# dahiyaaneesh/peclr

Measured on AMD Instinct MI355X. Metric: images/sec (2-view) ResNet-50 bs128 @1/2/4/8 MI355X; NT-Xent loss Δ vs ref, higher is better.
Workload: dtype fp32; 1 GPU; ResNet-50 encoder, 2x128 synthetic 224x224 views per GPU, crop+rotate equivariance alignment, NT-Xent tau=0.5, LARS(Adam) step, fp32; global_batch=256, parallelism=dp1, accumulate_grad_batches=1, launch=one hipGraph replay per step (whole step captured), bn=per-rank batch statistics

## Files before the change

peclr_amd/csrc/stem.hip:

```cpp
#include <stdlib.h>

#include <type_traits>

#include "mfma.hpp"

namespace peclr {
namespace {

constexpr int SK = 14;
constexpr int TPX = 128;
constexpr int PWP = 2 * TPX + 6;
constexpr int PROW = PWP * 8;
constexpr int NROW = 9;
constexpr int XE = 68;

struct StemArgs {
    const float* x;
    const void* planes;
    void* y;
    int N, Hin, Win, Ho, Wo;
    int tiles_w;
    const float* stat_shift;
    float* stat_partial;
};

struct X6 {
    static constexpr int NP = 3;
    typedef float Out;
    static __device__ __forceinline__ f32x16 mma(const uint4& a, const uint4& b, f32x16 acc) { return mma_bf16(a, b, acc); }
};
struct HB : BF16 {
    static constexpr int NP = 1;
    typedef h16_t Out;
};
struct HF : F16 {
    static constexpr int NP = 1;
    typedef h16_t Out;
};

template <typename F>
__global__ __launch_bounds__(256, 2) void stem_fwd_kernel(StemArgs g) {
    constexpr int NP = F::NP;
    constexpr int PLANE = NROW * PROW;
    constexpr int CH = NP * 2 * 1024;
    constexpr int NB = 4;
    constexpr int B0 = 0, P0 = NB * CH;
    constexpr int EPI = 4 * 32 * XE * 4 + 4 * 2 * 64 * 4;
    constexpr int TOTAL = P0 + NP * PLANE > EPI ? P0 + NP * PLANE : EPI;
    __shared__ __attribute__((aligned(1024))) unsigned char lds[TOTAL];
    const int tid = threadIdx.x, lane = tid & 63, wave = tid >> 6;
    const int i = lane & 31, half = lane >> 5;
    typedef __attribute__((address_space(3))) unsigned char* lptr_t;
    const unsigned lds0 = __builtin_amdgcn_readfirstlane((unsigned)(__UINTPTR_TYPE__)(lptr_t)lds);
    const int wave_s = __builtin_amdgcn_readfirstlane(wave);

// ... 150 lines not shown
#pragma unroll
        for (int y = 0; y < 2; ++y)
#pragma unroll
            for (int r = 0; r < 16; ++r) wl[mfma32_row(r, half) * XE + y * 32 + i] = acc[a][y][r];
#pragma unroll
        for (int jj = 0; jj < 4; ++jj) {
            const int ow = wpx0 + er + 8 * jj;
            const float4 c0 = *reinterpret_cast<const float4*>(wl + (er + 8 * jj) * XE + ec);
            const float4 c1 = *reinterpret_cast<const float4*>(wl + (er + 8 * jj) * XE + ec + 4);
            if (oh < g.Ho && ow < g.Wo) {
                const size_t o = (((size_t)img * g.Ho + oh) * g.Wo + ow) * 64 + ec;
                if constexpr (NP == 3) {
                    float* out = static_cast<float*>(g.y) + o;
                    *reinterpret_cast<float4*>(out) = c0;
                    *reinterpret_cast<float4*>(out + 4) = c1;
                } else {
                    uint16_t* out = static_cast<uint16_t*>(g.y) + o;
                    *reinterpret_cast<uint4*>(out) = make_uint4(F::pack2(c0.x, c0.y), F::pack2(c0.z, c0.w), F::pack2(c1.x, c1.y), F::pack2(c1.z, c1.w));
                }
            }
        }
    }
}

__global__ __launch_bounds__(128) void stem_pack_kernel(const float* w, long sn, long sc, long sh, long sw, unsigned char* planes, int fmt) {
    const int t = blockIdx.x, y = threadIdx.x >> 6, l = threadIdx.x & 63;
    const int n = 32 * y + (l & 31), slice = 2 * t + (l >> 5), kh = slice >> 2, s = slice & 3;
    float v[8];
#pragma unroll
    for (int kk = 0; kk < 8; ++kk) {
        const int kw = 2 * s + (kk >> 2), c = kk & 3;
        v[kk] = (kw < 7 && c < 3) ? w[n * sn + c * sc + kh * sh + kw * sw] : 0.f;
    }
    if (fmt == 0) {
        unsigned h[4], m[4], lo[4];
#pragma unroll
        for (int q = 0; q < 4; ++q) split3_pk(v[2 * q], v[2 * q + 1], h[q], m[q], lo[q]);
        unsigned char* d = planes + (size_t)t * 6144 + (y * 3) * 1024 + l * 16;
        *reinterpret_cast<uint4*>(d) = make_uint4(h[0], h[1], h[2], h[3]);
        *reinterpret_cast<uint4*>(d + 1024) = make_uint4(m[0], m[1], m[2], m[3]);
        *reinterpret_cast<uint4*>(d + 2048) = make_uint4(lo[0], lo[1], lo[2], lo[3]);
    } else {
        unsigned q4[4];
#pragma unroll
        for (int q = 0; q < 4; ++q) q4[q] = fmt == 2 ? HF::pack2(v[2 * q], v[2 * q + 1]) : HB::pack2(v[2 * q], v[2 * q + 1]);
        *reinterpret_cast<uint4*>(planes + (size_t)t * 2048 + y * 1024 + l * 16) = make_uint4(q4[0], q4[1], q4[2], q4[3]);
    }
}


constexpr int WPX = 64;
constexpr int WPW = 2 * WPX + 6;
constexpr int WROW = WPW * 8;
constexpr int WAP = (WPX + 8) * 2;

struct StemWArgs {
    const float* x;
    const void* dy;
    float* slabs;
    int N, Hin, Win, Ho, Wo, tiles_w;
    long long tiles;
    int abl;
};

struct Gather {
    unsigned lo[4], hi[4];
};
template <int OFF>
__device__ __forceinline__ void gather8(unsigned addr, Gather& r) {
    asm volatile(
        "ds_read_u16 %0, %8 offset:%9\n\t"
        "ds_read_u16 %4, %8 offset:%10\n\t"
        "ds_read_u16 %1, %8 offset:%11\n\t"
        "ds_read_u16 %5, %8 offset:%12\n\t"
        "ds_read_u16 %2, %8 offset:%13\n\t"
        "ds_read_u16 %6, %8 offset:%14\n\t"
        "ds_read_u16 %3, %8 offset:%15\n\t"
        "ds_read_u16 %7, %8 offset:%16"
        : "=v"(r.lo[0]), "=v"(r.lo[1]), "=v"(r.lo[2]), "=v"(r.lo[3]), "=v"(r.hi[0]), "=v"(r.hi[1]), "=v"(r.hi[2]), "=v"(r.hi[3])
        : "v"(addr), "n"(OFF), "n"(OFF + 16), "n"(OFF + 32), "n"(OFF + 48), "n"(OFF + 64), "n"(OFF + 80), "n"(OFF + 96), "n"(OFF + 112)
        : "memory");
}
template <int NP>
__device__ __forceinline__ void gather_fence(Gather (&g)[NP]) {
    if constexpr (NP == 3) {
        asm volatile("s_waitcnt lgkmcnt(0)"
                     : "+v"(g[0].lo[0]), "+v"(g[0].lo[1]), "+v"(g[0].lo[2]), "+v"(g[0].lo[3]), "+v"(g[0].hi[0]), "+v"(g[0].hi[1]),
                       "+v"(g[0].hi[2]), "+v"(g[0].hi[3]), "+v"(g[1].lo[0]), "+v"(g[1].lo[1]), "+v"(g[1].lo[2]), "+v"(g[1].lo[3]),
                       "+v"(g[1].hi[0]), "+v"(g[1].hi[1]), "+v"(g[1].hi[2]), "+v"(g[1].hi[3]), "+v"(g[2].lo[0]), "+v"(g[2].lo[1]),
                       "+v"(g[2].lo[2]), "+v"(g[2].lo[3]), "+v"(g[2].hi[0]), "+v"(g[2].hi[1]), "+v"(g[2].hi[2]), "+v"(g[2].hi[3])
                     :: "memory");
    } else {
        asm volatile("s_waitcnt lgkmcnt(0)"
                     : "+v"(g[0].lo[0]), "+v"(g[0].lo[1]), "+v"(g[0].lo[2]), "+v"(g[0].lo[3]), "+v"(g[0].hi[0]), "+v"(g[0].hi[1]),
                       "+v"(g[0].hi[2]), "+v"(g[0].hi[3])
                     :: "memory");
    }
}
__device__ __forceinline__ uint4 merge(const Gather& g) {
    return make_uint4(g.lo[0] | (g.hi[0] << 16), g.lo[1] | (g.hi[1] << 16), g.lo[2] | (g.hi[2] << 16), g.lo[3] | (g.hi[3] << 16));
}

template <typename F>
__global__ __launch_bounds__(256, F::NP == 3 ? 2 : 3) void stem_wgrad_kernel(StemWArgs g) {
    constexpr int NP = F::NP;
    constexpr int PPL = 7 * WROW;
    constexpr int APL = 64 * WAP;
    constexpr int STAGE = NP * (PPL + APL);
    constexpr int NST = NP == 3 ? 1 : 2;
    __shared__ __attribute__((aligned(16))) unsigned char lds[NST * STAGE];
    const int tid = threadIdx.x, lane = tid & 63, wave = tid >> 6;
    const int i = lane & 31, half = lane >> 5;
    typedef __attribute__((address_space(3))) unsigned char* lptr_t;
    const unsigned lds0 = (unsigned)(__UINTPTR_TYPE__)(lptr_t)lds;
    const int nkh = wave == 3 ? 1 : 2;

    f32x16 acc[2][2];
#pragma unroll
    for (int a = 0; a < 2; ++a)
#pragma unroll
        for (int b = 0; b < 2; ++b)
#pragma unroll
            for (int r = 0; r < 16; ++r) acc[a][b][r] = 0.f;

    constexpr int NSLOT = 7 * WPW, NLD = (NSLOT + 255) / 256;
    struct __attribute__((packed, aligned(4))) Rgb { float r, g, b; };
    Rgb pxs[2][NLD];
    constexpr int NDY = NP == 3 ? 4 : 2;
    uint4 dyrs[2][NDY];
    auto tile_of = [&](long long t64, int& img, int& oh, int& ow0) {
        const int per_img = g.Ho * g.tiles_w, t = (int)t64;
        img = t / per_img;
        const int rem = t - img * per_img;
        oh = rem / g.tiles_w;
        ow0 = (rem - oh * g.tiles_w) * WPX;
    };
    auto gload = [&](long long t, Rgb (&px)[NLD], uint4 (&dyr)[NDY]) {
        int img, oh, ow0;
        tile_of(t, img, oh, ow0);
        const int ih0 = 2 * oh - 3, iw0 = 2 * ow0 - 3;
#pragma unroll
        for (int u = 0; u < NLD; ++u) {
            const int idx = tid + 256 * u;
            const int r = idx / WPW, p = idx - r * WPW;
            const int ih = ih0 + r, iw = iw0 + p;
            const bool in = idx < NSLOT && (unsigned)ih < (unsigned)g.Hin && (unsigned)iw < (unsigned)g.Win;
            const Rgb* src = reinterpret_cast<const Rgb*>(g.x + (((size_t)img * g.Hin + (in ? ih : 0)) * g.Win + (in ? iw : 0)) * 3);
            px[u] = (in && !(g.abl & 16)) ? *src : Rgb{0.f, 0.f, 0.f};
        }
        const size_t row0 = ((size_t)img * g.Ho + oh) * g.Wo;
#pragma unroll
        for (int u = 0; u < NDY; ++u) {
            const int p = NP == 3 ? 16 * u + (lane & 15) : 32 * u + (lane & 31);
            const int grp = NP == 3 ? 4 * wave + (lane >> 4) : 2 * wave + (lane >> 5);
            const bool live = ow0 + p < g.Wo;
            const size_t row = row0 + (live ? ow0 + p : 0);
            const uint4* src = NP == 3 ? reinterpret_cast<const uint4*>(static_cast<const float*>(g.dy) + row * 64 + 4 * grp)
                                       : reinterpret_cast<const uint4*>(static_cast<const uint16_t*>(g.dy) + row * 64 + 8 * grp);
            if (live && !(g.abl & 1)) {
                if (g.abl & 32) {
                    const u32x4 t = __builtin_nontemporal_load(reinterpret_cast<const u32x4*>(src));
                    dyr[u] = make_uint4(t[0], t[1], t[2], t[3]);
                } else dyr[u] = *src;
            } else dyr[u] = make_uint4(0u, 0u, 0u, 0u);
        }
    };
    auto stage_store = [&](int st, const Rgb (&px)[NLD], const uint4 (&dyr)[NDY]) {
        unsigned char* base = lds + st * STAGE;
#pragma unroll
        for (int u = 0; u < NLD; ++u) {
            const int idx = tid + 256 * u;
            if (idx < NSLOT) {
                unsigned char* d = base + idx * 8;
                if constexpr (NP == 3) {
                    unsigned h[2], m[2], l[2];
                    split3_pk(px[u].r, px[u].g, h[0], m[0], l[0]);
                    split3_pk(px[u].b, 0.f, h[1], m[1], l[1]);
                    *reinterpret_cast<uint2*>(d) = make_uint2(h[0], h[1]);
                    *reinterpret_cast<uint2*>(d + PPL) = make_uint2(m[0], m[1]);
                    *reinterpret_cast<uint2*>(d + 2 * PPL) = make_uint2(l[0], l[1]);
                } else {
                    *reinterpret_cast<uint2*>(d) = make_uint2(F::pack2(px[u].r, px[u].g), F::pack2(px[u].b, 0.f));
                }
            }
        }
        unsigned char* ab = base + NP * PPL;
        if (g.abl & 2) return;
#pragma unroll
        for (int u = 0; u < NDY; ++u) {
            const int p = NP == 3 ? 16 * u + (lane & 15) : 32 * u + (lane & 31);
            const int grp = NP == 3 ? 4 * wave + (lane >> 4) : 2 * wave + (lane >> 5);
            if constexpr (NP == 3) {
                const unsigned w[4] = {dyr[u].x, dyr[u].y, dyr[u].z, dyr[u].w};
                unsigned h[2], m[2], l[2];
                split3_pk(__uint_as_float(w[0]), __uint_as_float(w[1]), h[0], m[0], l[0]);
                split3_pk(__uint_as_float(w[2]), __uint_as_float(w[3]), h[1], m[1], l[1]);
#pragma unroll
                for (int q = 0; q < 4; ++q) {
                    unsigned short* d = reinterpret_cast<unsigned short*>(ab + (4 * grp + q) * WAP + p * 2);
                    const int sh = (q & 1) * 16;
                    d[0] = (unsigned short)(h[q >> 1] >> sh);
                    d[APL / 2] = (unsigned short)(m[q >> 1] >> sh);
                    d[APL] = (unsigned short)(l[q >> 1] >> sh);
                }
            } else {
                const unsigned w[4] = {dyr[u].x, dyr[u].y, dyr[u].z, dyr[u].w};
#pragma unroll
                for (int q = 0; q < 8; ++q)
                    *reinterpret_cast<unsigned short*>(ab + (8 * grp + q) * WAP + p * 2) = (unsigned short)(w[q >> 1] >> ((q & 1) * 16));
            }
        }
    };

    const unsigned bbase = 2 * i + 128 * half + (2 * wave) * WROW;
    const unsigned abase = NP * PPL + i * WAP + 16 * half;

    auto products = [&](int st) {
        const unsigned sb = lds0 + st * STAGE;
        const unsigned char* sa = lds + st * STAGE + abase;
#pragma unroll
        for (int ks = 0; ks < WPX / 16; ++ks) {
            uint4 af[2][NP], bf[2][NP];
            Gather gb[2][NP];
#pragma unroll
            for (int p = 0; p < NP; ++p)
#pragma unroll
                for (int q = 0; q < 4; ++q) gb[1][p].lo[q] = gb[1][p].hi[q] = 0u;
#pragma unroll
            for (int mt = 0; mt < 2; ++mt)
#pragma unroll
                for (int p = 0; p < NP; ++p) af[mt][p] = *reinterpret_cast<const uint4*>(sa + p * APL + mt * 32 * WAP + ks * 32);
            auto row = [&](auto kc, int b) {
                constexpr int KO = decltype(kc)::value * 256;
                const unsigned addr = sb + bbase + b * WROW;
                gather8<KO>(addr, gb[b][0]);
                if constexpr (NP == 3) {
                    gather8<PPL + KO>(addr, gb[b][1]);
                    gather8<2 * PPL + KO>(addr, gb[b][2]);
                }
            };
            auto both = [&](auto kc) { row(kc, 0); if (nkh == 2) row(kc, 1); };
            if (g.abl & 4) { }
            else if (ks == 0) both(std::integral_constant<int, 0>{});
            else if (ks == 1) both(std::integral_constant<int, 1>{});
            else if (ks == 2) both(std::integral_constant<int, 2>{});
            else both(std::integral_constant<int, 3>{});
            gather_fence<NP>(gb[0]);
            gather_fence<NP>(gb[1]);
#pragma unroll
            for (int b = 0; b < 2; ++b)
#pragma unroll
                for (int p = 0; p < NP; ++p) bf[b][p] = merge(gb[b][p]);
#pragma unroll
            for (int b = 0; b < 2; ++b) {
                if (b < nkh && !(g.abl & 8)) {
#pragma unroll
                    for (int mt = 0; mt < 2; ++mt) {
                        if constexpr (NP == 3) {
                            acc[mt][b] = F::mma(af[mt][2], bf[b][0], acc[mt][b]);
                            acc[mt][b] = F::mma(af[mt][0], bf[b][2], acc[mt][b]);
                            acc[mt][b] = F::mma(af[mt][1], bf[b][1], acc[mt][b]);
                            acc[mt][b] = F::mma(af[mt][1], bf[b][0], acc[mt][b]);
                            acc[mt][b] = F::mma(af[mt][0], bf[b][1], acc[mt][b]);
                            acc[mt][b] = F::mma(af[mt][0], bf[b][0], acc[mt][b]);
                        } else {
                            acc[mt][b] = F::mma(af[mt][0], bf[b][0], acc[mt][b]);
                        }
                    }
                }
            }
        }
    };
    const long long step = gridDim.x;
    long long t = blockIdx.x;
    if (t < g.tiles) {
        gload(t, pxs[0], dyrs[0]);
        if (t + step < g.tiles) gload(t + step, pxs[1], dyrs[1]);
        stage_store(0, pxs[0], dyrs[0]);
    }
    __syncthreads();
    int st = 0;
    while (t < g.tiles) {
#pragma unroll
        for (int cur = 1; cur >= 0; --cur) {
            if (t < g.tiles) {
                if (t + 2 * step < g.tiles) gload(t + 2 * step, pxs[cur ^ 1], dyrs[cur ^ 1]);
                products(st);
                if constexpr (NST == 1) __syncthreads();
                if (t + step < g.tiles) stage_store(st ^ (NST - 1), pxs[cur], dyrs[cur]);
                __syncthreads();
                t += step;
                st ^= (NST - 1);
            }
        }
    }
    float* slab = g.slabs + (size_t)blockIdx.x * 64 * 224;
#pragma unroll
    for (int b = 0; b < 2; ++b) {
        if (b < nkh) {
            const int kh = 2 * wave + b;
#pragma unroll
            for (int mt = 0; mt < 2; ++mt)
#pragma unroll
                for (int r = 0; r < 16; ++r) slab[(size_t)(32 * mt + mfma32_row(r, half)) * 224 + 32 * kh + i] = acc[mt][b][r];
        }
// ... 81 lines not shown
```

peclr_amd/csrc/gemm_x6t.hip:

```cpp
#include "mfma.hpp"

#include <type_traits>

namespace peclr {
namespace {

constexpr int TK = 16;

struct X6TArgs {
    const float* A;
    const float* B;
    float* slabs;
    int M, N, K, lda, ldb, ldc;
    int kchunk;
    int taps, H, W;
    int stride;
    const float* zeros;
};

__device__ __forceinline__ int slot_of(int i) { return (i & 3) * 8 + ((i >> 2) ^ (((i >> 1) & 1) << 2)); }

template <int MT, int NT, int WGM, bool GEO, int PF>
__global__ __launch_bounds__(512, 2) void gemm_x6t_kernel(X6TArgs g) {
    constexpr int WGN = 8 / WGM;
// ... 245 lines not shown
        split_store(0);
        if (nk > 1) gload(1);
    }
    __syncthreads();
    for (int t = 0; t < nk; ++t) {
        const unsigned char* bufp = lds + (t & 1) * BUF;
        uint4 af[3];
#pragma unroll
        for (int p = 0; p < 3; ++p) af[p] = *reinterpret_cast<const uint4*>(bufp + fa + p * 2048);
#pragma unroll
        for (int tp = 0; tp < NACC; ++tp) {
            if (WGM == 4 || tp < ntap) {
                uint4 bf[3];
#pragma unroll
                for (int p = 0; p < 3; ++p) bf[p] = *reinterpret_cast<const uint4*>(bufp + fb + tp * GRP + p * 2048);
                acc[tp] = mma_bf16(af[2], bf[0], acc[tp]);
                acc[tp] = mma_bf16(af[0], bf[2], acc[tp]);
                acc[tp] = mma_bf16(af[1], bf[1], acc[tp]);
                acc[tp] = mma_bf16(af[1], bf[0], acc[tp]);
                acc[tp] = mma_bf16(af[0], bf[1], acc[tp]);
                acc[tp] = mma_bf16(af[0], bf[0], acc[tp]);
            }
            if (tp == (WGM == 4 ? 2 : 1) && t + 1 < nk) {
                if constexpr (!(ABL & 4)) split_store((t + 1) & 1);
                if constexpr (!(ABL & 8)) if (t + 2 < nk) gload(t + 2);
            }
        }
        __syncthreads();
    }

    float* out = g.slabs + (size_t)blockIdx.y * g.M * g.ldc;
    float* wlds = reinterpret_cast<float*>(lds) + wave * (32 * XEPL);
    const int er = lane >> 3, ec = (lane & 7) * 4;
    const int mt = m0 + wm * 32, nt = n0 + wn * 32;
#pragma unroll
    for (int tp = 0; tp < NACC; ++tp) {
        if (WGM != 4 && tp >= ntap) break;
#pragma unroll
        for (int r = 0; r < 16; ++r) wlds[mfma32_row(r, kh) * XEPL + i] = acc[tp][r];
#pragma unroll
        for (int jj = 0; jj < 4; ++jj) {
            const int m = mt + er + 8 * jj, n = nt + ec;
            const float4 c = *reinterpret_cast<const float4*>(wlds + (er + 8 * jj) * XEPL + ec);
            if (m < g.M && n < g.N) *reinterpret_cast<float4*>(out + (size_t)m * g.ldc + (tap0 + tp) * g.N + n) = c;
        }
    }
}

constexpr int X6W2_MAX_HW = 3136;
constexpr int X6W2_TAB = 9 * X6W2_MAX_HW + 192;
constexpr int X6W2_S2_MAX_HW = X6W2_TAB / 36 - 3;


template <int WGM, bool S2 = false>
__global__ __launch_bounds__(512, 2) void gemm_x6w2_kernel(X6TArgs g) {
    constexpr int GRP = 3 * 2 * 64 * 16;
    constexpr int NGA = WGM / 2, NG = NGA + 9, BUF = NG * GRP;
    constexpr int NACC = WGM == 4 ? 9 : 5;
    constexpr int XEPL = 36;
    __shared__ __attribute__((aligned(1024))) unsigned char lds[2 * BUF + X6W2_TAB];
    unsigned char* const tab = lds + 2 * BUF;
    const int tid = threadIdx.x, lane = tid & 63;
    const int wave = __builtin_amdgcn_readfirstlane(tid >> 6);
    const int wm = WGM == 4 ? wave >> 1 : (wave >> 1) & 1, wn = wave & 1;
    const int tap0 = WGM == 4 ? 0 : (wave >> 2) * 5;
    const int ntap = WGM == 4 ? 9 : (wave >> 2 ? 4 : 5);
    const int i = lane & 31, kh = lane >> 5;
    const int nct = (g.N + 63) / 64;
    const int m0 = (int)(blockIdx.x / nct) * (32 * WGM), n0 = (int)(blockIdx.x % nct) * 64;
    const int kbeg = blockIdx.y * g.kchunk, kend = min(g.K, kbeg + g.kchunk);
    const int nk = (kend - kbeg + TK - 1) / TK;
    const int HW = g.H * g.W;

    const unsigned s2_ld4 = (unsigned)g.ldb * 4u, s2_img = 4u * HW * s2_ld4;
    const int s2_row = (HW + 3) * 4;
    if constexpr (S2) {
        unsigned* t32 = reinterpret_cast<unsigned*>(tab);
        for (int p = tid; p < HW; p += 512) {
            const int oh = p / g.W, ow = p - oh * g.W;
#pragma unroll
            for (int tap = 0; tap < 9; ++tap) {
                const int ih = 2 * oh + tap / 3 - 1, iw = 2 * ow + tap % 3 - 1;
                const bool in = ih >= 0 && iw >= 0;
                const unsigned e = in ? (unsigned)(ih * 2 * g.W + iw) * s2_ld4 : 0x40000000u;
                t32[tap * (HW + 3) + p] = e;
                if (p < 3) t32[tap * (HW + 3) + HW + p] = in ? e + s2_img : 0x40000000u;
            }
        }
        __syncthreads();
    } else {

        unsigned short* pm = reinterpret_cast<unsigned short*>(lds);
        for (int p = tid; p < HW; p += 512) {
            const int oh = p / g.W, ow = p - oh * g.W;
            const unsigned rv = (oh > 0 ? 1u : 0u) | 2u | (oh + 1 < g.H ? 4u : 0u), cv = (ow > 0 ? 1u : 0u) | 2u | (ow + 1 < g.W ? 4u : 0u);
            unsigned bits = 0;
#pragma unroll
            for (int tap = 0; tap < 9; ++tap) bits |= ((rv >> (tap / 3)) & (cv >> (tap % 3)) & 1u) << tap;
            pm[p] = (unsigned short)bits;
        }
        __syncthreads();
        for (int p = tid; p < HW; p += 512) {
            unsigned v[4];
#pragma unroll
            for (int q = 0; q < 4; ++q) v[q] = pm[p + q < HW ? p + q : p + q - HW];
#pragma unroll
            for (int tap = 0; tap < 9; ++tap)
                tab[tap * X6W2_MAX_HW + p] = (unsigned char)(((v[0] >> tap) & 1u) | ((v[1] >> tap) & 1u) << 1 | ((v[2] >> tap) & 1u) << 2 | ((v[3] >> tap) & 1u) << 3);
        }
        __syncthreads();
    }

    const int chunk = (lane & 7) + 8 * (lane >> 5), kq = (lane >> 3) & 3;
    const int cin = 4 * (chunk & 7), tile = chunk >> 3;
    const int st_off = (kq >> 1) * 1024 + tile * 512 + (kq & 1) * 8;
    struct Grp {
        __amdgpu_buffer_rsrc_t rs;
        unsigned off;
        unsigned step, ld4;
        int tb;
        int st;
        bool isx;
    };
    auto grp_of = [&](int gi) {
        Grp s;
        const bool is_a = gi < NGA;
        const int tap = is_a ? 4 : gi - NGA;
        const int shift = (tap / 3 - 1) * g.W + (tap % 3 - 1);
        const int ld = is_a ? g.lda : g.ldb;
        const int c = 4 * chunk + (is_a ? 64 * gi : 0);
        const bool ok = is_a ? m0 + c < g.M : n0 + c < g.N;
        const long rows = S2 ? (is_a ? (long)g.K : 4L * g.K) : (long)g.K + (shift < 0 ? shift : 0);
        const unsigned long long bp = reinterpret_cast<unsigned long long>(is_a ? g.A : g.B);
        const unsigned blo = __builtin_amdgcn_readfirstlane((unsigned)bp), bhi = __builtin_amdgcn_readfirstlane((unsigned)(bp >> 32));
        s.rs = __builtin_amdgcn_make_buffer_rsrc(reinterpret_cast<void*>((unsigned long long)bhi << 32 | blo), (short)0,
                                                 __builtin_amdgcn_readfirstlane((int)(rows * ld * 4)), 0x00020000);
        s.ld4 = __builtin_amdgcn_readfirstlane((unsigned)ld * 4u);
        s.step = TK * s.ld4;
        s.off = ok ? (unsigned)(((kbeg + 4 * kq + shift) * ld + (is_a ? m0 : n0) + c) * 4) : 0x80000000u;
        s.tb = __builtin_amdgcn_readfirstlane(2 * BUF + tap * X6W2_MAX_HW);
        s.isx = !is_a;
        if constexpr (S2) {
            if (!is_a) s.off = ok ? (unsigned)((kbeg + 4 * kq) / HW) * s2_img + (unsigned)(n0 + c) * 4u : 0x80000000u;
            s.tb = __builtin_amdgcn_readfirstlane(2 * BUF + tap * s2_row);
        }
        s.st = gi * GRP + st_off;
        return s;
    };
    Grp G1 = grp_of(wave), G2 = grp_of(wave + 8 < NG ? wave + 8 : wave);
    const bool two = wave + 8 < NG;
    int pk = (kbeg + 4 * kq) % HW;

    f32x4 la[4], lb[4];
    unsigned m1 = 0, m2 = 0;
    auto issue_row = [&](const Grp& G, unsigned msk, int q, f32x4 (&r)[4]) {
        unsigned o;
        if constexpr (S2) o = G.off + (G.isx ? msk : q * G.ld4);
        else o = (msk >> q) & 1u ? G.off + q * G.ld4 : 0x80000000u;
        r[q] = __builtin_bit_cast(f32x4, __builtin_amdgcn_raw_buffer_load_b128(G.rs, (int)o, 0, 0));
    };
    auto entry = [&](const Grp& G, int q) { return *reinterpret_cast<const unsigned*>(lds + G.tb + 4 * (pk + q)); };
    auto issue = [&](const Grp& G, unsigned msk, int qp, f32x4 (&r)[4]) {
        if constexpr (S2) {
            issue_row(G, entry(G, 2 * qp), 2 * qp, r);
            issue_row(G, entry(G, 2 * qp + 1), 2 * qp + 1, r);
        } else {
            issue_row(G, msk, 2 * qp, r);
            issue_row(G, msk, 2 * qp + 1, r);
        }
    };
    unsigned winc = 0;
    auto next_pixel = [&]() {
        pk += TK;
        if constexpr (S2) winc = pk >= HW ? s2_img : 0u;
        pk = pk >= HW ? pk - HW : pk;
    };
    auto advance = [&](Grp& G) {
        if constexpr (S2) G.off += G.isx ? winc : G.step;
        else G.off += G.step;
    };
    struct Quarter { unsigned h, m; float r0, r1; };
    auto q_first = [&](Quarter& s, int qp, int j, const f32x4 (&r)[4]) {
        const float x0 = r[2 * qp][j], x1 = r[2 * qp + 1][j];
        s.h = pk_bf16(x0, x1);
        s.r0 = sub_f32(x0, __uint_as_float(s.h << 16));
        s.r1 = sub_f32(x1, __uint_as_float(s.h & 0xFFFF0000u));
    };
    auto q_second = [&](Quarter& s) {
        s.m = pk_bf16(s.r0, s.r1);
        s.r0 = sub_f32(s.r0, __uint_as_float(s.m << 16));
        s.r1 = sub_f32(s.r1, __uint_as_float(s.m & 0xFFFF0000u));
    };
    auto q_third = [&](const Quarter& s, const Grp& G, int buf, int qp, int j) {
        unsigned char* d = lds + G.st + buf * BUF + 4 * qp + slot_of(cin + j) * 16;
        *reinterpret_cast<unsigned*>(d) = s.h;
        *reinterpret_cast<unsigned*>(d + 2048) = s.m;
        *reinterpret_cast<unsigned*>(d + 4096) = pk_bf16(s.r0, s.r1);
    };
    auto quarter = [&](const Grp& G, int buf, int qp, int j, const f32x4 (&r)[4]) {
        Quarter s;
        q_first(s, qp, j, r);
        q_second(s);
        q_third(s, G, buf, qp, j);
    };

    f32x16 acc[NACC];
#pragma unroll
    for (int tp = 0; tp < NACC; ++tp)
#pragma unroll
        for (int r = 0; r < 16; ++r) acc[tp][r] = 0.f;
    const int fa = (wm >> 1) * GRP + kh * 1024 + (wm & 1) * 512 + slot_of(i) * 16;
    const int fb = (NGA + tap0) * GRP + kh * 1024 + wn * 512 + slot_of(i) * 16;

    __syncthreads();
    if constexpr (!S2) { m1 = lds[G1.tb + pk]; m2 = lds[G2.tb + pk]; }
    issue(G1, m1, 0, la); issue(G1, m1, 1, la);
    if (two) { issue(G2, m2, 0, lb); issue(G2, m2, 1, lb); }
    next_pixel(); advance(G1); advance(G2);
#pragma unroll
    for (int qp = 0; qp < 2; ++qp)
#pragma unroll
        for (int j = 0; j < 4; ++j) {
            quarter(G1, 0, qp, j, la);
            if (two) quarter(G2, 0, qp, j, lb);
        }
    if constexpr (!S2) { m1 = lds[G1.tb + pk]; m2 = lds[G2.tb + pk]; }
    issue(G1, m1, 0, la); issue(G1, m1, 1, la);
    if (two) { issue(G2, m2, 0, lb); issue(G2, m2, 1, lb); }
    next_pixel(); advance(G1); advance(G2);
    __syncthreads();

    auto run = [&](auto two_c) {
        constexpr bool TWO = decltype(two_c)::value;
        for (int t = 0; t < nk; ++t) {
            const unsigned char* bufp = lds + (t & 1) * BUF;
            const int nb = (t + 1) & 1;
            uint4 af[3], b0[2], b1, b2;
#pragma unroll
            for (int p = 0; p < 3; ++p) af[p] = *reinterpret_cast<const uint4*>(bufp + fa + p * 2048);
            b0[0] = *reinterpret_cast<const uint4*>(bufp + fb);
            b1 = *reinterpret_cast<const uint4*>(bufp + fb + 2048);
            b2 = *reinterpret_cast<const uint4*>(bufp + fb + 4096);
            const unsigned n1 = S2 ? 0u : lds[G1.tb + pk], n2 = (!S2 && TWO) ? lds[G2.tb + pk] : 0u;
            unsigned tq[2] = {0u, 0u};
#pragma unroll
            for (int tp = 0; tp < NACC; ++tp) {
                if (WGM != 4 && tp >= ntap) break;
                const int cb = tp & 1;
                const bool more = tp + 1 < NACC;
                const unsigned char* nx = bufp + fb + (tp + 1) * GRP;
                constexpr int PER = WGM == 4 ? 2 : 4;
                Quarter qs[PER];
                auto piece = [&](int e) {
                    const int u = PER * tp + e / 3, k = e % 3;
                    if (u >= (TWO ? 16 : 8)) return;
                    const int qp = (u >> 2) & 1, j = u & 3;
                    Quarter& s = qs[e / 3];
                    if (u < 8) {
                        if (k == 0) { q_first(s, qp, j, la); if (S2 && j == 2) { tq[0] = entry(G1, 2 * qp); tq[1] = entry(G1, 2 * qp + 1); } }
                        else if (k == 1) { q_second(s); if (j == 3) issue_row(G1, S2 ? tq[0] : n1, 2 * qp, la); }
                        else { q_third(s, G1, nb, qp, j); if (j == 3) issue_row(G1, S2 ? tq[1] : n1, 2 * qp + 1, la); }
                    } else {
                        if (k == 0) { q_first(s, qp, j, lb); if (S2 && j == 2) { tq[0] = entry(G2, 2 * qp); tq[1] = entry(G2, 2 * qp + 1); } }
                        else if (k == 1) { q_second(s); if (j == 3) issue_row(G2, S2 ? tq[0] : n2, 2 * qp, lb); }
                        else { q_third(s, G2, nb, qp, j); if (j == 3) issue_row(G2, S2 ? tq[1] : n2, 2 * qp + 1, lb); }
                    }
                };
                auto slot = [&](int si) {
                    if (WGM == 4) piece(si);
                    else { piece(2 * si); piece(2 * si + 1); }
                };
#define PECLR_FENCE __builtin_amdgcn_sched_barrier(0)
                acc[tp] = mma_bf16(af[2], b0[cb], acc[tp]);       PECLR_FENCE;
                if (more) b0[cb ^ 1] = *reinterpret_cast<const uint4*>(nx);
                slot(0);                                      PECLR_FENCE;
                acc[tp] = mma_bf16(af[0], b2, acc[tp]);           PECLR_FENCE;
                if (more) b2 = *reinterpret_cast<const uint4*>(nx + 4096);
                slot(1);                                      PECLR_FENCE;
                acc[tp] = mma_bf16(af[1], b1, acc[tp]);           PECLR_FENCE;
                slot(2);                                      PECLR_FENCE;
                acc[tp] = mma_bf16(af[1], b0[cb], acc[tp]);       PECLR_FENCE;
                slot(3);                                      PECLR_FENCE;
                acc[tp] = mma_bf16(af[0], b1, acc[tp]);           PECLR_FENCE;
                if (more) b1 = *reinterpret_cast<const uint4*>(nx + 2048);
                slot(4);                                      PECLR_FENCE;
                acc[tp] = mma_bf16(af[0], b0[cb], acc[tp]);       PECLR_FENCE;
                slot(5);                                      PECLR_FENCE;
#undef PECLR_FENCE
            }
            next_pixel();
            advance(G1);
            if (TWO) advance(G2);
            __syncthreads();
        }
    };
    if (two) run(std::true_type{});
    else run(std::false_type{});

    float* out = g.slabs + (size_t)blockIdx.y * g.M * g.ldc;
    float* wlds = reinterpret_cast<float*>(lds) + wave * (32 * XEPL);
    const int er = lane >> 3, ec = (lane & 7) * 4;
    const int mt = m0 + wm * 32, nt = n0 + wn * 32;
#pragma unroll
    for (int tp = 0; tp < NACC; ++tp) {
        if (WGM != 4 && tp >= ntap) break;
#pragma unroll
        for (int r = 0; r < 16; ++r) wlds[mfma32_row(r, kh) * XEPL + i] = acc[tp][r];
#pragma unroll
        for (int jj = 0; jj < 4; ++jj) {
            const int m = mt + er + 8 * jj, n = nt + ec;
            const float4 c = *reinterpret_cast<const float4*>(wlds + (er + 8 * jj) * XEPL + ec);
            if (m < g.M && n < g.N) *reinterpret_cast<float4*>(out + (size_t)m * g.ldc + (tap0 + tp) * g.N + n) = c;
        }
    }
}

template <int MT, int NT, int WGM, bool PF2 = false>
__global__ __launch_bounds__(512, 2) void gemm_x6t2_kernel(X6TArgs g) {
    constexpr int WGN = 8 / WGM;
    constexpr int TM = 32 * WGM * MT, TN = 32 * WGN * NT;
    static_assert((TM + TN) / 64 <= 8 && TM % 64 == 0 && TN % 64 == 0, "one 64-column group of the split per wave");
    constexpr int HALF_A = TM * 16, HALF_B = TN * 16;
    constexpr int PL_A = 2 * HALF_A, PL_B = 2 * HALF_B;
    constexpr int BUF = 3 * (PL_A + PL_B);
    constexpr int XEPL = 36;
    static_assert(2 * BUF >= 8 * 32 * XEPL * 4, "epilogue transposes live in the plane buffers");
    __shared__ __attribute__((aligned(1024))) unsigned char lds[2 * BUF];
    const int tid = threadIdx.x, lane = tid & 63;
    const int wave = __builtin_amdgcn_readfirstlane(tid >> 6);
    const int wm = wave / WGN, wn = wave % WGN;
    const int i = lane & 31, kh = lane >> 5;
    const int nct = (g.N + TN - 1) / TN;
    const int m0 = (int)(blockIdx.x / nct) * TM, n0 = (int)(blockIdx.x % nct) * TN;
    const int kbeg = blockIdx.y * g.kchunk, kend = min(g.K, kbeg + g.kchunk);
    const int nk = (kend - kbeg + TK - 1) / TK;

    const bool is_a = wave < TM / 64;
    const bool active = wave < (TM + TN) / 64;
    const int cgrp = is_a ? wave : wave - TM / 64;
    const int chunk = (lane & 7) + 8 * (lane >> 5);
    const int kq = (lane >> 3) & 3;
    const int col = cgrp * 64 + 4 * chunk;
    const int ld = is_a ? g.lda : g.ldb;
    const bool col_ok = active && (is_a ? m0 + col < g.M : n0 + col < g.N);
    const int tile = col >> 5, cin = col & 31;
    const int st_base = (kq >> 1) * (is_a ? HALF_A : HALF_B) + tile * 512 + (kq & 1) * 8 + (is_a ? 0 : 3 * PL_A);
    const int st_plane = is_a ? PL_A : PL_B;
    const bool once = is_a ? nct == 1 : (int)gridDim.x == nct;

    const unsigned long long bp = reinterpret_cast<unsigned long long>(is_a ? g.A : g.B);
// ... 248 lines not shown
```

Baseline: 5697 images/sec.

## Use ds_read_tr16 transposed LDS reads for stem wgrad fragments

Replaces the per-element ds_read_u16 gathers and merge for the pixel (B) fragments with ds_read_b64_tr_b16 transposing loads. It also changes the dy staging layout to pixel-major rows, written with wide vector stores instead of scattered 16-bit stores, and re-pads the A pitch. The intent is to cut LDS instruction count and the cost of scattered stores in the stem weight-gradient kernel. It relies on the gfx950 transpose-read builtin and a new lane-to-fragment mapping that must match the MFMA operand layout exactly.

```diff
diff --git a/peclr_amd/csrc/stem.hip b/peclr_amd/csrc/stem.hip
--- a/peclr_amd/csrc/stem.hip
+++ b/peclr_amd/csrc/stem.hip
@@ -1,6 +1,4 @@
 #include <stdlib.h>
-
-#include <type_traits>
 
 #include "mfma.hpp"
 
@@ -257,7 +255,7 @@
 constexpr int WPX = 64;
 constexpr int WPW = 2 * WPX + 6;
 constexpr int WROW = WPW * 8;
-constexpr int WAP = (WPX + 8) * 2;
+constexpr int WAP = 64 * 2 + 64;
 
 struct StemWArgs {
     const float* x;
@@ -268,56 +266,25 @@
     int abl;
 };
 
-struct Gather {
-    unsigned lo[4], hi[4];
-};
-template <int OFF>
-__device__ __forceinline__ void gather8(unsigned addr, Gather& r) {
-    asm volatile(
-        "ds_read_u16 %0, %8 offset:%9\n\t"
-        "ds_read_u16 %4, %8 offset:%10\n\t"
-        "ds_read_u16 %1, %8 offset:%11\n\t"
-        "ds_read_u16 %5, %8 offset:%12\n\t"
-        "ds_read_u16 %2, %8 offset:%13\n\t"
-        "ds_read_u16 %6, %8 offset:%14\n\t"
-        "ds_read_u16 %3, %8 offset:%15\n\t"
-        "ds_read_u16 %7, %8 offset:%16"
-        : "=v"(r.lo[0]), "=v"(r.lo[1]), "=v"(r.lo[2]), "=v"(r.lo[3]), "=v"(r.hi[0]), "=v"(r.hi[1]), "=v"(r.hi[2]), "=v"(r.hi[3])
-        : "v"(addr), "n"(OFF), "n"(OFF + 16), "n"(OFF + 32), "n"(OFF + 48), "n"(OFF + 64), "n"(OFF + 80), "n"(OFF + 96), "n"(OFF + 112)
-        : "memory");
-}
-template <int NP>
-__device__ __forceinline__ void gather_fence(Gather (&g)[NP]) {
-    if constexpr (NP == 3) {
-        asm volatile("s_waitcnt lgkmcnt(0)"
-                     : "+v"(g[0].lo[0]), "+v"(g[0].lo[1]), "+v"(g[0].lo[2]), "+v"(g[0].lo[3]), "+v"(g[0].hi[0]), "+v"(g[0].hi[1]),
-                       "+v"(g[0].hi[2]), "+v"(g[0].hi[3]), "+v"(g[1].lo[0]), "+v"(g[1].lo[1]), "+v"(g[1].lo[2]), "+v"(g[1].lo[3]),
-                       "+v"(g[1].hi[0]), "+v"(g[1].hi[1]), "+v"(g[1].hi[2]), "+v"(g[1].hi[3]), "+v"(g[2].lo[0]), "+v"(g[2].lo[1]),
-                       "+v"(g[2].lo[2]), "+v"(g[2].lo[3]), "+v"(g[2].hi[0]), "+v"(g[2].hi[1]), "+v"(g[2].hi[2]), "+v"(g[2].hi[3])
-                     :: "memory");
-    } else {
-        asm volatile("s_waitcnt lgkmcnt(0)"
-                     : "+v"(g[0].lo[0]), "+v"(g[0].lo[1]), "+v"(g[0].lo[2]), "+v"(g[0].lo[3]), "+v"(g[0].hi[0]), "+v"(g[0].hi[1]),
-                       "+v"(g[0].hi[2]), "+v"(g[0].hi[3])
-                     :: "memory");
-    }
-}
-__device__ __forceinline__ uint4 merge(const Gather& g) {
-    return make_uint4(g.lo[0] | (g.hi[0] << 16), g.lo[1] | (g.hi[1] << 16), g.lo[2] | (g.hi[2] << 16), g.lo[3] | (g.hi[3] << 16));
+typedef short s16x4 __attribute__((ext_vector_type(4)));
+template <int PITCH>
+__device__ __forceinline__ uint4 tr_frag(const unsigned char* base) {
+    typedef __attribute__((address_space(3))) s16x4* lp;
+    const uint2 lo = __builtin_bit_cast(uint2, __builtin_amdgcn_ds_read_tr16_b64_v4i16((lp)(base)));
+    const uint2 hi = __builtin_bit_cast(uint2, __builtin_amdgcn_ds_read_tr16_b64_v4i16((lp)(base + 4 * PITCH)));
+    return make_uint4(lo.x, lo.y, hi.x, hi.y);
 }
 
 template <typename F>
 __global__ __launch_bounds__(256, F::NP == 3 ? 2 : 3) void stem_wgrad_kernel(StemWArgs g) {
     constexpr int NP = F::NP;
     constexpr int PPL = 7 * WROW;
-    constexpr int APL = 64 * WAP;
+    constexpr int APL = WPX * WAP;
     constexpr int STAGE = NP * (PPL + APL);
     constexpr int NST = NP == 3 ? 1 : 2;
     __shared__ __attribute__((aligned(16))) unsigned char lds[NST * STAGE];
     const int tid = threadIdx.x, lane = tid & 63, wave = tid >> 6;
     const int i = lane & 31, half = lane >> 5;
-    typedef __attribute__((address_space(3))) unsigned char* lptr_t;
-    const unsigned lds0 = (unsigned)(__UINTPTR_TYPE__)(lptr_t)lds;
     const int nkh = wave == 3 ? 1 : 2;
 
     f32x16 acc[2][2];
@@ -356,8 +323,8 @@
         const size_t row0 = ((size_t)img * g.Ho + oh) * g.Wo;
 #pragma unroll
         for (int u = 0; u < NDY; ++u) {
-            const int p = NP == 3 ? 16 * u + (lane & 15) : 32 * u + (lane & 31);
-            const int grp = NP == 3 ? 4 * wave + (lane >> 4) : 2 * wave + (lane >> 5);
+            const int p = NP == 3 ? 16 * u + 4 * wave + (lane >> 4) : 32 * u + 8 * wave + (lane >> 3);
+            const int grp = NP == 3 ? lane & 15 : lane & 7;
             const bool live = ow0 + p < g.Wo;
             const size_t row = row0 + (live ? ow0 + p : 0);
             const uint4* src = NP == 3 ? reinterpret_cast<const uint4*>(static_cast<const float*>(g.dy) + row * 64 + 4 * grp)
@@ -393,69 +360,44 @@
         if (g.abl & 2) return;
 #pragma unroll
         for (int u = 0; u < NDY; ++u) {
-            const int p = NP == 3 ? 16 * u + (lane & 15) : 32 * u + (lane & 31);
-            const int grp = NP == 3 ? 4 * wave + (lane >> 4) : 2 * wave + (lane >> 5);
+            const int p = NP == 3 ? 16 * u + 4 * wave + (lane >> 4) : 32 * u + 8 * wave + (lane >> 3);
+            const int grp = NP == 3 ? lane & 15 : lane & 7;
             if constexpr (NP == 3) {
                 const unsigned w[4] = {dyr[u].x, dyr[u].y, dyr[u].z, dyr[u].w};
                 unsigned h[2], m[2], l[2];
                 split3_pk(__uint_as_float(w[0]), __uint_as_float(w[1]), h[0], m[0], l[0]);
                 split3_pk(__uint_as_float(w[2]), __uint_as_float(w[3]), h[1], m[1], l[1]);
-#pragma unroll
-                for (int q = 0; q < 4; ++q) {
-                    unsigned short* d = reinterpret_cast<unsigned short*>(ab + (4 * grp + q) * WAP + p * 2);
-                    const int sh = (q & 1) * 16;
-                    d[0] = (unsigned short)(h[q >> 1] >> sh);
-                    d[APL / 2] = (unsigned short)(m[q >> 1] >> sh);
-                    d[APL] = (unsigned short)(l[q >> 1] >> sh);
-                }
+                unsigned char* d = ab + p * WAP + grp * 8;
+                *reinterpret_cast<uint2*>(d) = make_uint2(h[0], h[1]);
+                *reinterpret_cast<uint2*>(d + APL) = make_uint2(m[0], m[1]);
+                *reinterpret_cast<uint2*>(d + 2 * APL) = make_uint2(l[0], l[1]);
             } else {
-                const unsigned w[4] = {dyr[u].x, dyr[u].y, dyr[u].z, dyr[u].w};
-#pragma unroll
-                for (int q = 0; q < 8; ++q)
-                    *reinterpret_cast<unsigned short*>(ab + (8 * grp + q) * WAP + p * 2) = (unsigned short)(w[q >> 1] >> ((q & 1) * 16));
+                *reinterpret_cast<uint4*>(ab + p * WAP + grp * 16) = dyr[u];
             }
         }
     };
 
-    const unsigned bbase = 2 * i + 128 * half + (2 * wave) * WROW;
-    const unsigned abase = NP * PPL + i * WAP + 16 * half;
+    const int fpix = 8 * half + ((lane & 15) >> 2), fcol = 2 * (16 * ((lane >> 4) & 1) + 4 * (lane & 3));
+    const unsigned bbase = fpix * 16 + fcol + (2 * wave) * WROW;
+    const unsigned abase = NP * PPL + fpix * WAP + fcol;
 
     auto products = [&](int st) {
-        const unsigned sb = lds0 + st * STAGE;
+        const unsigned char* sb = lds + st * STAGE + bbase;
         const unsigned char* sa = lds + st * STAGE + abase;
 #pragma unroll
         for (int ks = 0; ks < WPX / 16; ++ks) {
             uint4 af[2][NP], bf[2][NP];
-            Gather gb[2][NP];
-#pragma unroll
-            for (int p = 0; p < NP; ++p)
-#pragma unroll
-                for (int q = 0; q < 4; ++q) gb[1][p].lo[q] = gb[1][p].hi[q] = 0u;
 #pragma unroll
             for (int mt = 0; mt < 2; ++mt)
 #pragma unroll
-                for (int p = 0; p < NP; ++p) af[mt][p] = *reinterpret_cast<const uint4*>(sa + p * APL + mt * 32 * WAP + ks * 32);
-            auto row = [&](auto kc, int b) {
-                constexpr int KO = decltype(kc)::value * 256;
-                const unsigned addr = sb + bbase + b * WROW;
-                gather8<KO>(addr, gb[b][0]);
-                if constexpr (NP == 3) {
-                    gather8<PPL + KO>(addr, gb[b][1]);
-                    gather8<2 * PPL + KO>(addr, gb[b][2]);
+                for (int p = 0; p < NP; ++p) af[mt][p] = tr_frag<WAP>(sa + p * APL + mt * 64 + ks * 16 * WAP);
+#pragma unroll
+            for (int b = 0; b < 2; ++b)
+#pragma unroll
+                for (int p = 0; p < NP; ++p) {
+                    bf[b][p] = make_uint4(0u, 0u, 0u, 0u);
+                    if (b < nkh && !(g.abl & 4)) bf[b][p] = tr_frag<16>(sb + p * PPL + b * WROW + ks * 256);
                 }
-            };
-            auto both = [&](auto kc) { row(kc, 0); if (nkh == 2) row(kc, 1); };
-            if (g.abl & 4) { }
-            else if (ks == 0) both(std::integral_constant<int, 0>{});
-            else if (ks == 1) both(std::integral_constant<int, 1>{});
-            else if (ks == 2) both(std::integral_constant<int, 2>{});
-            else both(std::integral_constant<int, 3>{});
-            gather_fence<NP>(gb[0]);
-            gather_fence<NP>(gb[1]);
-#pragma unroll
-            for (int b = 0; b < 2; ++b)
-#pragma unroll
-                for (int p = 0; p < NP; ++p) bf[b][p] = merge(gb[b][p]);
 #pragma unroll
             for (int b = 0; b < 2; ++b) {
                 if (b < nkh && !(g.abl & 8)) {
```

After: 5678 images/sec. Within noise of the previous version (-0.3%).

## Move x6w2 tile barrier before last tap and reorder global loads for coalescing

Applied to the files above, without the earlier changes.

Restructures the main loop of the 3x3 implicit-GEMM weight-gradient kernel so the per-tile __syncthreads and the next tile's LDS fragment preloads happen before the final tap's MFMAs rather than after all taps. The goal is to hide the barrier and the LDS reload latency behind compute. It also permutes which k-rows each lane loads and stores (XOR-swizzled row offsets and masks) so that global loads and LDS stores coalesce better. This adds complexity in the mask bit fixups and redistributes the conversion work across taps. There is a risk of correctness bugs and higher register pressure.

```diff
diff --git a/peclr_amd/csrc/gemm_x6t.hip b/peclr_amd/csrc/gemm_x6t.hip
--- a/peclr_amd/csrc/gemm_x6t.hip
+++ b/peclr_amd/csrc/gemm_x6t.hip
@@ -321,7 +321,13 @@
 constexpr int X6W2_S2_MAX_HW = X6W2_TAB / 36 - 3;
 
 
-template <int WGM, bool S2 = false>
+#ifndef PECLR_X6W2_EARLY_BARRIER
+#define PECLR_X6W2_EARLY_BARRIER 1
+#endif
+#ifndef PECLR_X6W2_CF_STORES
+#define PECLR_X6W2_CF_STORES 1
+#endif
+template <int WGM, bool S2 = false, bool EB = PECLR_X6W2_EARLY_BARRIER != 0, bool CF = PECLR_X6W2_CF_STORES != 0>
 __global__ __launch_bounds__(512, 2) void gemm_x6w2_kernel(X6TArgs g) {
     constexpr int GRP = 3 * 2 * 64 * 16;
     constexpr int NGA = WGM / 2, NG = NGA + 9, BUF = NG * GRP;
@@ -382,11 +388,13 @@
 
     const int chunk = (lane & 7) + 8 * (lane >> 5), kq = (lane >> 3) & 3;
     const int cin = 4 * (chunk & 7), tile = chunk >> 3;
-    const int st_off = (kq >> 1) * 1024 + tile * 512 + (kq & 1) * 8;
+    const int qx = CF ? kq & 2 : 0;
+    const int st_off = (kq >> 1) * 1024 + tile * 512 + (kq & 1) * 8 + 2 * qx;
     struct Grp {
         __amdgpu_buffer_rsrc_t rs;
         unsigned off;
         unsigned step, ld4;
+        unsigned hop;
         int tb;
         int st;
         bool isx;
@@ -406,7 +414,8 @@
                                                  __builtin_amdgcn_readfirstlane((int)(rows * ld * 4)), 0x00020000);
         s.ld4 = __builtin_amdgcn_readfirstlane((unsigned)ld * 4u);
         s.step = TK * s.ld4;
-        s.off = ok ? (unsigned)(((kbeg + 4 * kq + shift) * ld + (is_a ? m0 : n0) + c) * 4) : 0x80000000u;
+        s.off = ok ? (unsigned)(((kbeg + 4 * kq + qx + shift) * ld + (is_a ? m0 : n0) + c) * 4) : 0x80000000u;
+        s.hop = qx ? 0u - 2u * s.ld4 : 2u * s.ld4;
         s.tb = __builtin_amdgcn_readfirstlane(2 * BUF + tap * X6W2_MAX_HW);
         s.isx = !is_a;
         if constexpr (S2) {
@@ -422,13 +431,20 @@
 
     f32x4 la[4], lb[4];
     unsigned m1 = 0, m2 = 0;
+    auto row_off = [&](const Grp& G, int q) {
+        if constexpr (CF) return G.off + (q & 1) * G.ld4 + (q >> 1 ? G.hop : 0u);
+        else return G.off + q * G.ld4;
+    };
+    auto mask_raw = [&](const Grp& G) { return (unsigned)lds[G.tb + pk]; };
+    auto mask_fix = [&](unsigned m) { return CF ? (m | m << 4) >> qx : m; };
+    auto mask_of = [&](const Grp& G) { return mask_fix(mask_raw(G)); };
     auto issue_row = [&](const Grp& G, unsigned msk, int q, f32x4 (&r)[4]) {
         unsigned o;
-        if constexpr (S2) o = G.off + (G.isx ? msk : q * G.ld4);
-        else o = (msk >> q) & 1u ? G.off + q * G.ld4 : 0x80000000u;
+        if constexpr (S2) o = G.isx ? G.off + msk : row_off(G, q);
+        else o = (msk >> q) & 1u ? row_off(G, q) : 0x80000000u;
         r[q] = __builtin_bit_cast(f32x4, __builtin_amdgcn_raw_buffer_load_b128(G.rs, (int)o, 0, 0));
     };
-    auto entry = [&](const Grp& G, int q) { return *reinterpret_cast<const unsigned*>(lds + G.tb + 4 * (pk + q)); };
+    auto entry = [&](const Grp& G, int q) { return *reinterpret_cast<const unsigned*>(lds + G.tb + 4 * (pk + (q ^ qx))); };
     auto issue = [&](const Grp& G, unsigned msk, int qp, f32x4 (&r)[4]) {
         if constexpr (S2) {
             issue_row(G, entry(G, 2 * qp), 2 * qp, r);
@@ -461,7 +477,7 @@
         s.r1 = sub_f32(s.r1, __uint_as_float(s.m & 0xFFFF0000u));
     };
     auto q_third = [&](const Quarter& s, const Grp& G, int buf, int qp, int j) {
-        unsigned char* d = lds + G.st + buf * BUF + 4 * qp + slot_of(cin + j) * 16;
+        unsigned char* d = CF ? lds + ((G.st + buf * BUF + slot_of(cin + j) * 16) ^ (4 * qp)) : lds + G.st + buf * BUF + 4 * qp + slot_of(cin + j) * 16;
         *reinterpret_cast<unsigned*>(d) = s.h;
         *reinterpret_cast<unsigned*>(d + 2048) = s.m;
         *reinterpret_cast<unsigned*>(d + 4096) = pk_bf16(s.r0, s.r1);
@@ -482,7 +498,7 @@
     const int fb = (NGA + tap0) * GRP + kh * 1024 + wn * 512 + slot_of(i) * 16;
 
     __syncthreads();
-    if constexpr (!S2) { m1 = lds[G1.tb + pk]; m2 = lds[G2.tb + pk]; }
+    if constexpr (!S2) { m1 = mask_of(G1); m2 = mask_of(G2); }
     issue(G1, m1, 0, la); issue(G1, m1, 1, la);
     if (two) { issue(G2, m2, 0, lb); issue(G2, m2, 1, lb); }
     next_pixel(); advance(G1); advance(G2);
@@ -493,38 +509,52 @@
             quarter(G1, 0, qp, j, la);
             if (two) quarter(G2, 0, qp, j, lb);
         }
-    if constexpr (!S2) { m1 = lds[G1.tb + pk]; m2 = lds[G2.tb + pk]; }
+    if constexpr (!S2) { m1 = mask_of(G1); m2 = mask_of(G2); }
     issue(G1, m1, 0, la); issue(G1, m1, 1, la);
     if (two) { issue(G2, m2, 0, lb); issue(G2, m2, 1, lb); }
     next_pixel(); advance(G1); advance(G2);
     __syncthreads();
 
-    auto run = [&](auto two_c) {
+    auto run = [&](auto two_c, auto nt_c) {
         constexpr bool TWO = decltype(two_c)::value;
+        constexpr int NT = decltype(nt_c)::value;
+        constexpr int NP = 3 * (TWO ? 16 : 8);
+        constexpr int PPT = WGM == 4 ? (EB && TWO ? 7 : 6) : 12;
+        static_assert(!EB || NP <= PPT * (NT - 1), "the plane stores must end before the last tap");
+        auto frag = [&](const unsigned char* p) { return *reinterpret_cast<const uint4*>(p); };
+        uint4 af[4], b0[2], b1, b2;
+        unsigned n1 = 0u, n2 = 0u;
+        if constexpr (EB) {
+            af[0] = frag(lds + fa); af[1] = frag(lds + fa + 2048); af[2] = frag(lds + fa + 4096);
+            b0[0] = frag(lds + fb); b1 = frag(lds + fb + 2048); b2 = frag(lds + fb + 4096);
+            if constexpr (!S2) { n1 = mask_of(G1); if (TWO) n2 = mask_of(G2); }
+        }
         for (int t = 0; t < nk; ++t) {
-            const unsigned char* bufp = lds + (t & 1) * BUF;
-            const int nb = (t + 1) & 1;
-            uint4 af[3], b0[2], b1, b2;
-#pragma unroll
-            for (int p = 0; p < 3; ++p) af[p] = *reinterpret_cast<const uint4*>(bufp + fa + p * 2048);
-            b0[0] = *reinterpret_cast<const uint4*>(bufp + fb);
-            b1 = *reinterpret_cast<const uint4*>(bufp + fb + 2048);
-            b2 = *reinterpret_cast<const uint4*>(bufp + fb + 4096);
-            const unsigned n1 = S2 ? 0u : lds[G1.tb + pk], n2 = (!S2 && TWO) ? lds[G2.tb + pk] : 0u;
+            const int cur = t & 1, nb = cur ^ 1;
+            const unsigned char* bufp = lds + cur * BUF;
+            const unsigned char* nxb = lds + nb * BUF;
+            if constexpr (!EB) {
+#pragma unroll
+                for (int p = 0; p < 3; ++p) af[p] = frag(bufp + fa + p * 2048);
+                b0[0] = frag(bufp + fb);
+                b1 = frag(bufp + fb + 2048);
+                b2 = frag(bufp + fb + 4096);
+                if constexpr (!S2) { n1 = mask_of(G1); if (TWO) n2 = mask_of(G2); }
+            }
             unsigned tq[2] = {0u, 0u};
-#pragma unroll
-            for (int tp = 0; tp < NACC; ++tp) {
-                if (WGM != 4 && tp >= ntap) break;
+            Quarter qs[2];
+#pragma unroll
+            for (int tp = 0; tp < NT; ++tp) {
+                if (!EB && WGM != 4 && tp >= ntap) break;
                 const int cb = tp & 1;
-                const bool more = tp + 1 < NACC;
+                const bool more = tp + 1 < NT;
+                const bool last = EB && tp + 1 == NT;
                 const unsigned char* nx = bufp + fb + (tp + 1) * GRP;
-                constexpr int PER = WGM == 4 ? 2 : 4;
-                Quarter qs[PER];
                 auto piece = [&](int e) {
-                    const int u = PER * tp + e / 3, k = e % 3;
-                    if (u >= (TWO ? 16 : 8)) return;
+                    const int u = e / 3, k = e % 3;
+                    if (e >= NP) return;
                     const int qp = (u >> 2) & 1, j = u & 3;
-                    Quarter& s = qs[e / 3];
+                    Quarter& s = qs[u & 1];
                     if (u < 8) {
                         if (k == 0) { q_first(s, qp, j, la); if (S2 && j == 2) { tq[0] = entry(G1, 2 * qp); tq[1] = entry(G1, 2 * qp + 1); } }
                         else if (k == 1) { q_second(s); if (j == 3) issue_row(G1, S2 ? tq[0] : n1, 2 * qp, la); }
@@ -536,35 +566,64 @@
                     }
                 };
                 auto slot = [&](int si) {
-                    if (WGM == 4) piece(si);
-                    else { piece(2 * si); piece(2 * si + 1); }
+#pragma unroll
+                    for (int e = si * PPT / 6; e < (si + 1) * PPT / 6; ++e) piece(PPT * tp + e);
                 };
 #define PECLR_FENCE __builtin_amdgcn_sched_barrier(0)
+                if (last) {
+                    next_pixel();
+                    advance(G1);
+                    if (TWO) advance(G2);
+                    __syncthreads();
+                    b0[cb ^ 1] = frag(nxb + fb);
+                    af[3] = frag(nxb + fa);
+                    if constexpr (!S2) { n1 = mask_raw(G1); if (TWO) n2 = mask_raw(G2); }
+                    PECLR_FENCE;
+                }
                 acc[tp] = mma_bf16(af[2], b0[cb], acc[tp]);       PECLR_FENCE;
-                if (more) b0[cb ^ 1] = *reinterpret_cast<const uint4*>(nx);
+                if (more) b0[cb ^ 1] = frag(nx);
+                if (last) af[2] = frag(nxb + fa + 4096);
                 slot(0);                                      PECLR_FENCE;
                 acc[tp] = mma_bf16(af[0], b2, acc[tp]);           PECLR_FENCE;
-                if (more) b2 = *reinterpret_cast<const uint4*>(nx + 4096);
+                if (more) b2 = frag(nx + 4096);
+                if (last) b2 = frag(nxb + fb + 4096);
                 slot(1);                                      PECLR_FENCE;
                 acc[tp] = mma_bf16(af[1], b1, acc[tp]);           PECLR_FENCE;
                 slot(2);                                      PECLR_FENCE;
                 acc[tp] = mma_bf16(af[1], b0[cb], acc[tp]);       PECLR_FENCE;
+                if (last) af[1] = frag(nxb + fa + 2048);
                 slot(3);                                      PECLR_FENCE;
                 acc[tp] = mma_bf16(af[0], b1, acc[tp]);           PECLR_FENCE;
-                if (more) b1 = *reinterpret_cast<const uint4*>(nx + 2048);
+                if (more) b1 = frag(nx + 2048);
+                if (last) b1 = frag(nxb + fb + 2048);
                 slot(4);                                      PECLR_FENCE;
                 acc[tp] = mma_bf16(af[0], b0[cb], acc[tp]);       PECLR_FENCE;
                 slot(5);                                      PECLR_FENCE;
 #undef PECLR_FENCE
             }
-            next_pixel();
-            advance(G1);
-            if (TWO) advance(G2);
-            __syncthreads();
-        }
-    };
-    if (two) run(std::true_type{});
-    else run(std::false_type{});
+            if constexpr (!EB) {
+                next_pixel();
+                advance(G1);
+                if (TWO) advance(G2);
+                __syncthreads();
+            } else {
+                af[0] = af[3];
+                if (NT & 1) b0[0] = b0[1];
+                if constexpr (!S2) { n1 = mask_fix(n1); if (TWO) n2 = mask_fix(n2); }
+            }
+        }
+    };
+    if constexpr (!EB) {
+        if (two) run(std::true_type{}, std::integral_constant<int, NACC>{});
+        else run(std::false_type{}, std::integral_constant<int, NACC>{});
+    } else if constexpr (WGM == 4) {
+        if (two) run(std::true_type{}, std::integral_constant<int, 9>{});
+        else run(std::false_type{}, std::integral_constant<int, 9>{});
+    } else {
+        if (two) run(std::true_type{}, std::integral_constant<int, 5>{});
+        else if (ntap == 5) run(std::false_type{}, std::integral_constant<int, 5>{});
+        else run(std::false_type{}, std::integral_constant<int, 4>{});
+    }
 
     float* out = g.slabs + (size_t)blockIdx.y * g.M * g.ldc;
     float* wlds = reinterpret_cast<float*>(lds) + wave * (32 * XEPL);
```

After: 5693 images/sec before, 5707 images/sec after (median of 4 runs). Within noise of the previous version (+0.2%).
